# GZHoffie/approximate-string-matching

Measured on AMD Instinct MI355X. Metric: alignments/sec (1e6-pair batch, 100bp, err=0.10) per GPU; NW penalty bit-exact %, higher is better.
Workload: dtype u64; 1 GPU; C2: 1000000 pairs per GPU, len 100-100, err 0.10, k=3, x=o=e=1,1,1, aligners nw+leap+greedy, greedy tails=clean; pairs_per_gpu=1000000

## Files before the change

### approximate-string-matching_amd/csrc/asm_capi.hip

```cpp
#include <hip/hip_runtime.h>
#include <hipcub/hipcub.hpp>
#include <math.h>
#include <stddef.h>
#include <stdio.h>
#include <stdlib.h>
#include <string.h>

#include <algorithm>
#include <atomic>
#include <chrono>
#include <condition_variable>
#include <fcntl.h>
#include <functional>
#include <map>
#include <memory>
#include <mutex>
#include <string>
#include <sys/stat.h>
#include <thread>
#include <type_traits>
#include <unistd.h>
#include <unordered_map>
#include <vector>

#include "../../include/asm_mi355x.h"
#include "asm_host.h"
#include "asm_kernels.h"
#include "asm_greedy3_kernel.h"
#include "asm_wide.h"
#include "asm_wave.h"
#include "asm_group.h"
#include "asm_cover.h"
#include "asm_tails.h"
#include "asm_filter.h"
#include "asm_ingest.h"
#include "asm_map.h"
#include "asm_fastq.h"
#include "asm_sam.h"

struct asm_handle {
    unsigned long long serial = 0;
    int device = 0;
    hipStream_t own_stream = nullptr;
    hipStream_t stream = nullptr;
    unsigned long long* d_pair_queue = nullptr;
    hipStream_t side_stream = nullptr;
    hipStream_t pack_stream = nullptr;
    hipEvent_t ev_packed = nullptr;
    hipEvent_t ev_nw = nullptr;
    hipStream_t acc_stream = nullptr;
    hipEvent_t ev_leap = nullptr, ev_tail = nullptr;
    bool tail_set = false;
    hipEvent_t ev_out[2] = {nullptr, nullptr};
    unsigned calls3 = 0;
    const void* last3_out[3] = {nullptr, nullptr, nullptr};
    bool last3_valid = false;
    bool pipe_prev = false;
    hipEvent_t ev_gate = nullptr;
    bool gate_set = false;
    hipEvent_t ev_fork = nullptr, ev_join = nullptr, ev_switch = nullptr;
    bool overlap = true;
    std::string err;
    int num_cus = 256;
    int refill_greedy = 8;
    bool greedy_fast = true;
    struct G3Table {
        G3Sig sig;
        int k;
        bool ok;
        uint2* d;
    };
    std::vector<G3Table> g3_tables;
    const uint2* d_g3_table = nullptr;
    bool leap_hint = true;
    bool bucketing = true;
    bool wave_kernels = true;
    bool nw_bylen = true;
    bool nw_banded = true;
    bool nw_wfa = true;
    int64_t map_cand_cap = (int64_t)1 << 24;
    int64_t map_chunk = (int64_t)1 << 18;
    int64_t map_run_cap = (int64_t)1 << 24;
    std::vector<hipEvent_t> prof_ev;
    std::vector<unsigned> prof_mask;
    int prof_cap = 0;
    unsigned prof_select = 0xfu;
    void* d_sort = nullptr;
    size_t sort_cap = 0;
    bool leap_sort = true;
    uint32_t* d_todo = nullptr;
    size_t todo_cap = 0;
    std::unordered_map<void*, size_t> pool_live;
    std::multimap<size_t, void*> pool_idle;
    size_t pool_idle_bytes = 0;
    bool pooling = true;
    char* pin_raw[3] = {nullptr, nullptr, nullptr};
    size_t pin_raw_cap = 0;
    int32_t* pin_pen[2][3] = {{nullptr, nullptr, nullptr}, {nullptr, nullptr, nullptr}};
    int64_t pin_pen_cap[2][3] = {{0, 0, 0}, {0, 0, 0}};
};

static size_t pool_round(size_t bytes) {
    if (bytes <= 4096) return 4096;
    int top = 63 - __builtin_clzll((unsigned long long)bytes);
    const size_t step = (size_t)1 << (top - 3);
    return (bytes + step - 1) & ~(step - 1);
}
// ... 221 lines not shown
            hipStreamSynchronize(h->stream) == hipSuccess) {
            t.ok = true;
        } else {
            (void)hipGetLastError();
            if (t.d) (void)hipFree(t.d);
            t.d = nullptr;
        }
    }
    h->g3_tables.push_back(t);
    h->d_g3_table = t.d;
    return t.ok;
}

template <int K>
static hipError_t launch_greedy_fast(asm_handle* h, const asm_bucket& b, const GreedyArgs& ga, OutMap out, CigarSink cig) {
    constexpr int NT = G3_THREADS;
    auto kern = greedy_fast_kernel<K, NT>;
    const size_t lds = g3_lds_bytes(K, NT);
    {
        hipError_t e = hipFuncSetAttribute(reinterpret_cast<const void*>(kern), hipFuncAttributeMaxDynamicSharedMemorySize, (int)lds);
        if (e != hipSuccess) return e;
    }
    int64_t blocks = h->num_cus;
    const int64_t need = (b.n + NT - 1) / NT;
    if (blocks > need) blocks = need;
    const G3Sig sig = {ga.sig_match, ga.sig_mismatch, ga.sig_indel};
    hipLaunchKernelGGL(kern, dim3((unsigned)blocks), dim3(NT), lds, h->stream, (const uint4*)b.planes, (const uint32_t*)b.lens,
                       (long)b.n, b.w4, sig, h->d_g3_table, out, cig, h->refill_greedy);
    return hipGetLastError();
}

template <int K>
static hipError_t launch_greedy(asm_handle* h, const asm_bucket& b, const GreedyArgs& ga, OutMap out, CigarSink cig) {
#ifdef GREEDY_DIAG
    if (cig.ops == nullptr && g_diag_buf) cig.nops = (uint8_t*)g_diag_buf;
#endif
    const bool unit = ga.x == 1 && ga.o == 1 && ga.e == 1 && !ga.semi;
    if constexpr (K <= 3) {
        if (h->greedy_fast && unit && g3_prepare(h, ga, K)) return launch_greedy_fast<K>(h, b, ga, out, cig);
    }
    if (unit)
        return launch_persistent(h, greedy_persist_kernel<K, true>, b.n, (const uint4*)b.planes, (const uint32_t*)b.lens,
                                 (long)b.n, b.w4, ga, out, cig, h->refill_greedy);
    return launch_persistent(h, greedy_persist_kernel<K, false>, b.n, (const uint4*)b.planes, (const uint32_t*)b.lens,
                             (long)b.n, b.w4, ga, out, cig, h->refill_greedy);
}

#define LEAP_UNIT_WIDE_K 5
#define LEAP_UNIT_MAX_K 10
template <int K, int W64>
static hipError_t launch_leap_unit_w(asm_handle* h, const asm_bucket& b, OutMap out, const int32_t* hint) {
    if (hint && h->leap_hint) {
        const unsigned blocks = (unsigned)((b.n + LEAP_HINT_PAIRS - 1) / LEAP_HINT_PAIRS);
        hipLaunchKernelGGL((leap_unit_hint_kernel<K, W64>), dim3(blocks), dim3(ASM_BLOCK), 0, h->stream, b.planes, b.lens,
                           (long)b.n, b.w4, out, hint);
        return hipGetLastError();
    }
    hipLaunchKernelGGL((leap_unit_kernel<K, W64>), dim3(grid_for(b.n)), dim3(ASM_BLOCK), 0, h->stream, b.planes, b.lens,
                       (long)b.n, b.w4, out);
    return hipGetLastError();
}

template <int K, int W64>
static hipError_t launch_leap_general_w(asm_handle* h, const asm_bucket& b, const asm_params* p, OutMap out) {
    const dim3 grid((unsigned)((b.n + LEAP_GEN_THREADS - 1) / LEAP_GEN_THREADS)), block(LEAP_GEN_THREADS);
    const RingGeometry rg(p->x, p->o, p->e);
    const bool bytes = b.maxlen + 4 <= 255 && rg.lds_bytes(2 * K + 1, LEAP_GEN_THREADS, 2) > 20 * 1024;
    if (bytes)
        hipLaunchKernelGGL((leap_general_kernel<K, W64, uint8_t>), grid, block, rg.lds_bytes(2 * K + 1, LEAP_GEN_THREADS, 1), h->stream,
                           b.planes, b.lens, (long)b.n, b.w4, (int)p->x, (int)p->o, (int)p->e, rg.gm, rg.gi, out);
    else
        hipLaunchKernelGGL((leap_general_kernel<K, W64, uint16_t>), grid, block, rg.lds_bytes(2 * K + 1, LEAP_GEN_THREADS, 2), h->stream,
                           b.planes, b.lens, (long)b.n, b.w4, (int)p->x, (int)p->o, (int)p->e, rg.gm, rg.gi, out);
    return hipGetLastError();
}

template <int K, int W64, typename EnT>
static void launch_nw_wfa_pass(asm_handle* h, const asm_bucket& b, const asm_params* p, OutMap out, const uint32_t* in_list,
                               const uint32_t* in_count, uint32_t* todo, uint32_t* todo_count) {
    const WfaRings rg(p->x, p->o, p->e);
    const dim3 grid((unsigned)((b.n + LEAP_GEN_THREADS - 1) / LEAP_GEN_THREADS)), block(LEAP_GEN_THREADS);
    hipLaunchKernelGGL((nw_wfa_kernel<K, W64, EnT, false>), grid, block, rg.lds_bytes(2 * K + 1, LEAP_GEN_THREADS, sizeof(EnT)),
                       h->stream, b.planes, b.lens, (long)b.n, b.w4, (int)p->x, (int)p->o, (int)p->e, rg.gm, rg.gi, out, in_list,
                       in_count, todo, todo_count);
}

template <int W64, int MAXROWS>
static int launch_nw_wfa(asm_handle* h, const asm_bucket& b, const asm_params* p, OutMap out) {
    const size_t words = 2 * ((size_t)b.n + 1);
    if (h->todo_cap < words) {
        if (h->d_todo) (void)hipFree(h->d_todo);
        h->d_todo = nullptr, h->todo_cap = 0;
        HIPCHK(h, big_malloc(h, (void**)&h->d_todo, sizeof(uint32_t) * words));
        h->todo_cap = words;
    }
    uint32_t* const list_a = h->d_todo;
    uint32_t* const list_b = h->d_todo + (size_t)b.n + 1;
    HIPCHK(h, hipMemsetAsync(list_a, 0, sizeof(uint32_t), h->stream));
    HIPCHK(h, hipMemsetAsync(list_b, 0, sizeof(uint32_t), h->stream));
    const WfaRings rg(p->x, p->o, p->e);
    bool bytes = false;
    if constexpr (W64 == 2) {
        bytes = true;
        launch_nw_wfa_pass<NW_WFA_K, 2, uint8_t>(h, b, p, out, nullptr, nullptr, list_a + 1, list_a);
    }
    if (!bytes) launch_nw_wfa_pass<NW_WFA_K, W64, uint16_t>(h, b, p, out, nullptr, nullptr, list_a + 1, list_a);
    const uint32_t* rest = list_a;
    const size_t en = b.maxlen + 2 <= 255 ? 1 : 2;
// ... 127 lines not shown
        SIMD_ED_CASE(1)
        SIMD_ED_CASE(2)
        SIMD_ED_CASE(3)
        SIMD_ED_CASE(4)
        SIMD_ED_CASE(5)
        SIMD_ED_CASE(6)
        SIMD_ED_CASE(7)
        SIMD_ED_CASE(8)
        default: {
            const size_t lds = (size_t)2 * (2 * T + 3) * SIMD_ED_THREADS * sizeof(short);
            hipLaunchKernelGGL((simd_ed_kernel<0, W64>), grid, block, lds, h->stream, b.planes, b.lens, (long)b.n, b.w4, T, shd,
                               ed_mode, ev);
        }
    }
#undef SIMD_ED_CASE
    HIPCHK(h, hipGetLastError());
    return ASM_OK;
}

extern "C" {

const char* asm_version(void) { return "asm_mi355x 0.1 (gfx950)"; }

void asm_default_params(asm_params* p) {
    if (!p) return;
    p->k = 3;
    p->x = p->o = p->e = 1;
    p->p_match = 0.80;
    p->p_mismatch = 0.20 / 3;
    p->p_indel = 0.40 / 3;
    p->alignment_type = ASM_ALIGN_GLOBAL;
    p->leap_mode = ASM_LEAP_GLOBAL;
}

int asm_device_count(void) {
    int c = 0;
    if (hipGetDeviceCount(&c) != hipSuccess) return 0;
    return c;
}

static void handle_teardown(asm_handle* h) {
    (void)hipSetDevice(h->device);
    if (h->own_stream) (void)hipStreamDestroy(h->own_stream);
    if (h->side_stream) (void)hipStreamDestroy(h->side_stream);
    if (h->d_pair_queue) (void)hipFree(h->d_pair_queue);
    if (h->d_sort) (void)hipFree(h->d_sort);
    if (h->pack_stream) (void)hipStreamDestroy(h->pack_stream);
    if (h->ev_packed) (void)hipEventDestroy(h->ev_packed);
    if (h->ev_gate) (void)hipEventDestroy(h->ev_gate);
    if (h->ev_leap) (void)hipEventDestroy(h->ev_leap);
    if (h->ev_tail) (void)hipEventDestroy(h->ev_tail);
    for (hipEvent_t ev : h->ev_out)
        if (ev) (void)hipEventDestroy(ev);
    if (h->acc_stream) (void)hipStreamDestroy(h->acc_stream);
    if (h->ev_nw) (void)hipEventDestroy(h->ev_nw);
    if (h->ev_fork) (void)hipEventDestroy(h->ev_fork);
    if (h->ev_join) (void)hipEventDestroy(h->ev_join);
    if (h->ev_switch) (void)hipEventDestroy(h->ev_switch);
    if (h->d_todo) (void)hipFree(h->d_todo);
    for (auto& t : h->g3_tables)
        if (t.d) (void)hipFree(t.d);
    for (hipEvent_t ev : h->prof_ev) (void)hipEventDestroy(ev);
    (void)hipDeviceSynchronize();
    for (char* q : h->pin_raw)
        if (q) (void)hipHostFree(q);
    for (auto& row : h->pin_pen)
        for (int32_t* q : row)
            if (q) (void)hipHostFree(q);
    pool_release_idle(h);
    for (auto& kv : h->pool_live) (void)hipFree(kv.first);
    delete h;
}

int asm_create(asm_handle** out, int device) {
    if (!out) return fail(nullptr, ASM_EINVAL, "asm_create: out is NULL");
    *out = nullptr;
    int c = 0;
    if (hipGetDeviceCount(&c) != hipSuccess || c <= 0)
        return fail(nullptr, ASM_ENODEVICE, "asm_create: no HIP device is visible (this library has no CPU path)");
    if (device < 0 || device >= c) return fail(nullptr, ASM_EINVAL, "asm_create: device index out of range");
    std::unique_ptr<asm_handle, void (*)(asm_handle*)> owned(new asm_handle, handle_teardown);
    asm_handle* const h = owned.get();
    h->device = device;
    HIPCHK(h, hipSetDevice(device));
    HIPCHK(h, hipStreamCreateWithFlags(&h->own_stream, hipStreamNonBlocking));
    h->stream = h->own_stream;
    HIPCHK(h, hipStreamCreateWithFlags(&h->side_stream, hipStreamNonBlocking));
    HIPCHK(h, hipMalloc((void**)&h->d_pair_queue, sizeof(unsigned long long)));
    HIPCHK(h, hipStreamCreateWithFlags(&h->pack_stream, hipStreamNonBlocking));
    HIPCHK(h, hipEventCreateWithFlags(&h->ev_packed, hipEventDisableTiming));
    HIPCHK(h, hipEventCreateWithFlags(&h->ev_gate, hipEventDisableTiming));
    HIPCHK(h, hipStreamCreateWithFlags(&h->acc_stream, hipStreamNonBlocking));
    HIPCHK(h, hipEventCreateWithFlags(&h->ev_nw, hipEventDisableTiming));
    HIPCHK(h, hipEventCreateWithFlags(&h->ev_leap, hipEventDisableTiming));
    HIPCHK(h, hipEventCreateWithFlags(&h->ev_tail, hipEventDisableTiming));
    for (hipEvent_t& ev : h->ev_out) HIPCHK(h, hipEventCreateWithFlags(&ev, hipEventDisableTiming));
    HIPCHK(h, hipEventCreateWithFlags(&h->ev_fork, hipEventDisableTiming));
    HIPCHK(h, hipEventCreateWithFlags(&h->ev_join, hipEventDisableTiming));
    HIPCHK(h, hipEventCreateWithFlags(&h->ev_switch, hipEventDisableTiming));
    hipDeviceProp_t prop;
    HIPCHK(h, hipGetDeviceProperties(&prop, device));
    h->num_cus = prop.multiProcessorCount > 0 ? prop.multiProcessorCount : 256;
    const char* env;
    if ((env = getenv("ASM_OVERLAP"))) h->overlap = env[0] != '0';
    if ((env = getenv("ASM_LEAP_HINT"))) h->leap_hint = env[0] != '0';
    if ((env = getenv("ASM_LEAP_SORT"))) h->leap_sort = env[0] != '0';
    if ((env = getenv("ASM_BUCKET"))) h->bucketing = env[0] != '0';
    if ((env = getenv("ASM_WAVE"))) h->wave_kernels = env[0] != '0';
    if ((env = getenv("ASM_POOL"))) h->pooling = env[0] != '0';
    if ((env = getenv("ASM_NW_BANDED"))) h->nw_banded = env[0] != '0';
    if ((env = getenv("ASM_NW_BYLEN"))) h->nw_bylen = env[0] != '0';
    if ((env = getenv("ASM_NW_WFA"))) h->nw_wfa = env[0] != '0';
    if ((env = getenv("ASM_GREEDY_FAST"))) h->greedy_fast = env[0] != '0';
    if ((env = getenv("ASM_MAP_CAND_CAP")) && atoll(env) > 0) h->map_cand_cap = atoll(env);
    if ((env = getenv("ASM_MAP_CHUNK")) && atoll(env) > 0) h->map_chunk = atoll(env);
    if ((env = getenv("ASM_MAP_RUN_CAP")) && atoll(env) > 0) h->map_run_cap = atoll(env);
    {
        std::lock_guard<std::mutex> lk(g_live_mu);
        h->serial = g_next_serial++;
        g_live_handles.push_back(h);
    }
    *out = owned.release();
    return ASM_OK;
}

int asm_destroy(asm_handle* h) {
    if (!h) return ASM_OK;
    {
        std::lock_guard<std::mutex> lk(g_live_mu);
        for (size_t i = 0; i < g_live_handles.size(); i++)
            if (g_live_handles[i] == h) {
                g_live_handles.erase(g_live_handles.begin() + (long)i);
                break;
            }
    }
    handle_teardown(h);
    return ASM_OK;
}

const char* asm_last_error(const asm_handle* h) { return h ? h->err.c_str() : g_err.c_str(); }

static int switch_stream(asm_handle* h, hipStream_t next) {
    if (next == h->stream) return ASM_OK;
    HIPCHK(h, hipSetDevice(h->device));
    HIPCHK(h, hipEventRecord(h->ev_switch, h->stream));
    HIPCHK(h, hipStreamWaitEvent(next, h->ev_switch, 0));
    if (h->tail_set) HIPCHK(h, hipStreamWaitEvent(next, h->ev_tail, 0));
    h->stream = next;
    return ASM_OK;
}

int asm_set_stream(asm_handle* h, void* hip_stream) {
    if (!h) return fail(nullptr, ASM_EINVAL, "asm_set_stream: NULL handle");
    return switch_stream(h, (hipStream_t)hip_stream);
}

int asm_reset_stream(asm_handle* h) {
    if (!h) return fail(nullptr, ASM_EINVAL, "asm_reset_stream: NULL handle");
    return switch_stream(h, h->own_stream);
}

int asm_synchronize(asm_handle* h) {
    if (!h) return fail(nullptr, ASM_EINVAL, "asm_synchronize: NULL handle");
    HIPCHK(h, hipSetDevice(h->device));
    HIPCHK(h, hipStreamSynchronize(h->stream));
    if (h->tail_set) HIPCHK(h, hipStreamSynchronize(h->acc_stream));
    return ASM_OK;
}

int asm_pipeline_join_async(asm_handle* h) {
    if (!h) return fail(nullptr, ASM_EINVAL, "asm_pipeline_join_async: NULL handle");
    HIPCHK(h, hipSetDevice(h->device));
    if (h->tail_set) HIPCHK(h, hipStreamWaitEvent(h->stream, h->ev_tail, 0));
    h->pipe_prev = false;
    h->last3_valid = false;
    return ASM_OK;
}

static int check_gen(const asm_gen_config* cfg) {
    std::string err;
    const int rc = asm_host::check_gen(cfg, err);
    return rc ? fail(nullptr, rc, err) : ASM_OK;
}

int asm_generate_pairs(const asm_gen_config* cfg, int64_t first, int64_t n, uint32_t* read_off, uint32_t* ref_off,
                       char* reads, size_t reads_cap, char* refs, size_t refs_cap) {
    std::string err;
    const int rc = asm_host::generate_pairs(cfg, first, n, read_off, ref_off, reads, reads_cap, refs, refs_cap, err);
    return rc ? fail(nullptr, rc, err) : ASM_OK;
}


static hipError_t launch_pack(asm_handle* h, const asm_batch* b, const uint4* tails, uint4* planes, uint32_t* lens,
                              const PackBuckets& pb, const uint32_t* pos) {
    const dim3 grid((unsigned)((b->n + PACK_BLOCK - 1) / PACK_BLOCK)), block(PACK_BLOCK);
    int wmax = 1;
    for (int q = 0; q < pb.nb; q++) wmax = pb.w4[q] > wmax ? pb.w4[q] : wmax;
    const auto side_dwords = [](size_t bytes) { return (size_t)2 * (size_t)(((bytes + 15) / 16 + 1) / 2 + 1); };
    size_t dw = 2 * side_dwords((size_t)PACK_BLOCK * (size_t)b->maxlen + 15);
    if (dw > PACK_LDS_MAX / 4) dw = PACK_LDS_MAX / 4;
    if (dw < side_dwords((size_t)b->maxlen + 30)) dw = side_dwords((size_t)b->maxlen + 30);
#define PACK_LAUNCH(W)                                                                                                   \
    hipLaunchKernelGGL((pack_kernel<W>), grid, block, dw * 4, h->stream, b->d_reads, b->d_read_off, b->d_refs,           \
                       b->d_ref_off, tails, planes, lens, (long)b->n, pb, pos, (uint32_t)dw)
    switch (wmax) {
        case 1: PACK_LAUNCH(1); break;
        case 2: PACK_LAUNCH(2); break;
        case 3: PACK_LAUNCH(3); break;
        default: PACK_LAUNCH(4); break;
    }
#undef PACK_LAUNCH
    return hipGetLastError();
}

int asm_batch_pack_async(asm_handle* h, asm_batch* b) {
    if (!h || !b) return fail(h, ASM_EINVAL, "asm_batch_pack_async: NULL argument");
    if (b->n == 0) return ASM_OK;
    HIPCHK(h, hipSetDevice(h->device));
    HIPCHK(h, launch_pack(h, b, b->d_tails, b->d_planes, b->d_lens, b->pb, b->d_pos));
    return ASM_OK;
}

static int batch_resolve_tails(asm_handle* h, asm_batch* b, const uint8_t* init256, uint8_t* summary256, bool emit) {
    if (summary256) memset(summary256, TAIL_NONE, 256);
    if (b->n == 0) return ASM_OK;
    const long nchunks = (b->n + TAIL_CHUNK - 1) / TAIL_CHUNK;
// ... 341 lines not shown
        HIPCHK(h, hipMemcpy(refs, b->d_refs, b->refs_bytes, hipMemcpyDeviceToHost));
    }
    return ASM_OK;
}

int64_t asm_batch_planes_size(const asm_batch* b) { return b ? (int64_t)b->planes_total : 0; }

int asm_batch_download_planes(asm_handle* h, const asm_batch* b, uint32_t* planes, size_t planes_cap, uint32_t* lens,
                              uint32_t* order) {
    if (!h || !b) return fail(h, ASM_EINVAL, "asm_batch_download_planes: NULL argument");
    HIPCHK(h, hipSetDevice(h->device));
    HIPCHK(h, hipStreamSynchronize(h->stream));
    const size_t n = (size_t)b->n;
    if (planes) {
        if (planes_cap < 4 * b->planes_total) return fail(h, ASM_EINVAL, "asm_batch_download_planes: planes buffer too small");
        HIPCHK(h, hipMemcpy(planes, b->d_planes, sizeof(uint4) * b->planes_total, hipMemcpyDeviceToHost));
    }
    if (lens && n) HIPCHK(h, hipMemcpy(lens, b->d_lens, sizeof(uint32_t) * n, hipMemcpyDeviceToHost));
    if (order && n) {
        if (b->d_order) HIPCHK(h, hipMemcpy(order, b->d_order, sizeof(uint32_t) * n, hipMemcpyDeviceToHost));
        else
            for (size_t i = 0; i < n; i++) order[i] = (uint32_t)i;
    }
    return ASM_OK;
}

static int check_params(asm_handle* h, int aligner, const asm_params* p, int maxlen = ASM_MAX_LENGTH) {
    if (!p) return fail(h, ASM_EINVAL, "params is NULL");
    if (p->x < 0 || p->o < 0 || p->e < 0) return fail(h, ASM_EINVAL, "penalties must be non-negative");
    if (aligner == ASM_GREEDY) {
        if (p->k < 0 || p->k > ASM_GREEDY_MAX_K) return fail(h, ASM_EINVAL, "Greedy: k must be in [0, 50] (MAX_K, hurdle_matrix.h:8)");
        if (!(p->p_match > 0 && p->p_mismatch > 0 && p->p_indel > 0)) return fail(h, ASM_EINVAL, "Greedy: probabilities must be positive");
        if (p->alignment_type != ASM_ALIGN_GLOBAL && p->alignment_type != ASM_ALIGN_SEMI_GLOBAL)
            return fail(h, ASM_EUNSUPPORTED, "Greedy: alignment type must be GLOBAL or SEMI_GLOBAL (LOCAL is unsupported in the reference too, hurdle_matrix.h:467)");
    } else if (aligner == ASM_LEAP) {
        if (p->k < 0 || p->k > ASM_WIDE_MAX_K) return fail(h, ASM_EINVAL, "LEAP: k out of range");
        if (p->x < 1 || p->o < 1 || p->e < 1 || p->o < p->e)
            return fail(h, ASM_EINVAL, "LEAP: need x >= 1, o >= e >= 1 (LV_BAG.cpp:165-166)");
        if (p->x > ASM_WIDE_MAX_PENALTY || p->o > ASM_WIDE_MAX_PENALTY)
            return fail(h, ASM_EUNSUPPORTED, "LEAP: penalties above the compiled history depth");
        if (p->leap_mode < ASM_LEAP_GLOBAL || p->leap_mode > ASM_LEAP_SEMI_FREE_END)
            return fail(h, ASM_EINVAL, "LEAP: leap_mode must be one of ASM_LEAP_GLOBAL/LOCAL/SEMI_FREE_BEGIN/SEMI_FREE_END");
        if (p->leap_mode != ASM_LEAP_GLOBAL && maxlen > 512)
            return fail(h, ASM_EUNSUPPORTED, "LEAP: the non-GLOBAL modes are built for strings up to 512 characters");
    } else if (aligner == ASM_NW) {
        const long worst = 2L * ((long)p->o + (long)(maxlen > 0 ? maxlen - 1 : 0) * (long)p->e) + (long)p->o;
        if (p->x > 10000 || p->o > 10000 || p->e > 10000 || worst >= (long)NW_BIG)
            return fail(h, ASM_EUNSUPPORTED, "NW: penalties too large for this batch's longest sequence "
                                             "(need 2*(o + (maxlen-1)*e) + o < 30000 and x, o, e <= 10000)");
    } else {
        return fail(h, ASM_EINVAL, "unknown aligner id");
    }
    return ASM_OK;
}

static int align_bucket(asm_handle* h, const asm_bucket& b, int aligner, const asm_params* p, OutMap out,
                        CigarSink cig = CigarSink{nullptr, nullptr, 0}, const int32_t* hint = nullptr) {
    if (b.n == 0) return ASM_OK;
    const bool unit = (p->x == 1 && p->o == 1 && p->e == 1);
    const uint4* planes = b.planes;
    const uint32_t* lens = b.lens;
    if (aligner == ASM_GREEDY) {
        GreedyArgs ga;
        ga.x = p->x, ga.o = p->o, ga.e = p->e;
        ga.semi = p->alignment_type == ASM_ALIGN_SEMI_GLOBAL ? 1 : 0;
        ga.sig_match = log(p->p_match / 0.25);
        ga.sig_mismatch = log(p->p_mismatch / 0.25);
        ga.sig_indel = log(p->p_indel / 2 / 0.25);
        switch (p->k) {
            case 1: HIPCHK(h, launch_greedy<1>(h, b, ga, out, cig)); break;
            case 2: HIPCHK(h, launch_greedy<2>(h, b, ga, out, cig)); break;
            case 3: HIPCHK(h, launch_greedy<3>(h, b, ga, out, cig)); break;
            case 4: HIPCHK(h, launch_greedy<4>(h, b, ga, out, cig)); break;
            case 5: HIPCHK(h, launch_greedy<5>(h, b, ga, out, cig)); break;
#define GREEDY_WIDE_CASE(KK) \
            case KK: HIPCHK(h, launch_greedy<KK>(h, b, ga, out, cig)); break;
            GREEDY_WIDE_CASE(6) GREEDY_WIDE_CASE(7) GREEDY_WIDE_CASE(8) GREEDY_WIDE_CASE(9) GREEDY_WIDE_CASE(10) GREEDY_WIDE_CASE(11)
            GREEDY_WIDE_CASE(12) GREEDY_WIDE_CASE(13) GREEDY_WIDE_CASE(14) GREEDY_WIDE_CASE(15) GREEDY_WIDE_CASE(16)
#undef GREEDY_WIDE_CASE
            default:
                if (h->wave_kernels && p->k >= 32 && p->k <= 39 && (long)p->o + 110L * p->e < 16000L) {
                    HIPCHK(h, launch_greedy_group(h->stream, planes, lens, b.n, b.w4, (int)p->k, ga, out, cig, h->num_cus));
                } else if (p->k <= ASM_WAVE_MAX_K && h->wave_kernels && unit && !ga.semi) {
                    HIPCHK(h, hipMemsetAsync(h->d_pair_queue, 0, sizeof(unsigned long long), h->stream));
                    launch_wave_per_pair(h->stream, greedy_wave_kernel<true>, b.n, h->num_cus, planes, lens, (long)b.n, b.w4,
                                         (int)p->k, ga, out, cig, h->d_pair_queue, (const uint32_t*)nullptr, (const uint32_t*)nullptr);
                } else if (p->k <= ASM_WAVE_MAX_K && h->wave_kernels && (long)p->o + 62L * p->e < 16000L) {
                    HIPCHK(h, hipMemsetAsync(h->d_pair_queue, 0, sizeof(unsigned long long), h->stream));
                    launch_wave_per_pair(h->stream, greedy_wave_kernel<false>, b.n, h->num_cus, planes, lens, (long)b.n, b.w4,
                                         (int)p->k, ga, out, cig, h->d_pair_queue, (const uint32_t*)nullptr, (const uint32_t*)nullptr);
                } else if (h->wave_kernels && (long)p->o + 100L * p->e < 16000L)
                    launch_greedy_wave2(h->stream, planes, lens, b.n, b.w4, (int)p->k, ga, out, cig, h->num_cus);
                else
                    launch_greedy_wide(h->stream, planes, lens, b.n, b.w4, p->k, ga, out, cig);
                break;
        }
    } else if (aligner == ASM_LEAP) {
        if (p->leap_mode != ASM_LEAP_GLOBAL) {
            launch_leap_wide(h->stream, planes, lens, b.n, b.w4, p->k, p->x, p->o, p->e, out, (int)p->leap_mode);
        } else if (unit && p->k >= 1 && ((p->k <= LEAP_UNIT_WIDE_K && b.maxlen <= 384) || (p->k <= LEAP_UNIT_MAX_K && b.maxlen <= 128))) {
            switch (p->k) {
                case 1: HIPCHK(h, launch_leap_unit<1>(h, b, out, hint)); break;
                case 2: HIPCHK(h, launch_leap_unit<2>(h, b, out, hint)); break;
                case 3: HIPCHK(h, launch_leap_unit<3>(h, b, out, hint)); break;
                case 4: HIPCHK(h, launch_leap_unit<4>(h, b, out, hint)); break;
                case 5: HIPCHK(h, launch_leap_unit<5>(h, b, out, hint)); break;
                case 6: HIPCHK(h, launch_leap_unit<6>(h, b, out, hint)); break;
                case 7: HIPCHK(h, launch_leap_unit<7>(h, b, out, hint)); break;
                case 8: HIPCHK(h, launch_leap_unit<8>(h, b, out, hint)); break;
                case 9: HIPCHK(h, launch_leap_unit<9>(h, b, out, hint)); break;
                default: HIPCHK(h, launch_leap_unit<10>(h, b, out, hint)); break;
            }
        } else if (!unit && p->k >= 1 && ((p->k <= 5 && b.maxlen <= 256) || (p->k <= 8 && b.maxlen <= 128)) && h->wave_kernels &&
                   RingGeometry(p->x, p->o, p->e).lds_bytes(2 * p->k + 1, LEAP_GEN_THREADS) <= 64 * 1024) {
            switch (p->k) {
                case 1: HIPCHK(h, launch_leap_general<1>(h, b, p, out)); break;
                case 2: HIPCHK(h, launch_leap_general<2>(h, b, p, out)); break;
                case 3: HIPCHK(h, launch_leap_general<3>(h, b, p, out)); break;
                case 4: HIPCHK(h, launch_leap_general<4>(h, b, p, out)); break;
                case 5: HIPCHK(h, launch_leap_general<5>(h, b, p, out)); break;
                case 6: HIPCHK(h, launch_leap_general<6>(h, b, p, out)); break;
                case 7: HIPCHK(h, launch_leap_general<7>(h, b, p, out)); break;
                default: HIPCHK(h, launch_leap_general<8>(h, b, p, out)); break;
            }
        } else if (h->wave_kernels && b.maxlen <= 512 &&
                   leap_quad_lds((b.maxlen + 31) / 32, (int)p->k, unit ? 2 : RingGeometry(p->x, p->o, p->e).gm,
                                 unit ? 0 : RingGeometry(p->x, p->o, p->e).gi, b.maxlen + 2 <= 255 ? 1 : 2) <= 64 * 1024) {
            const RingGeometry rg(p->x, p->o, p->e);
            const int w32 = (b.maxlen + 31) / 32;
            const int32_t* const qhint = h->leap_hint ? hint : nullptr;
            const uint32_t* qperm = nullptr;
            if (qhint && h->leap_sort && (b.maxlen > 128 || !unit)) {
                const size_t n = (size_t)b.n;
                size_t tmp_bytes = 0;
                HIPCHK(h, hipcub::DeviceRadixSort::SortPairs(nullptr, tmp_bytes, (uint8_t*)nullptr, (uint8_t*)nullptr, (uint32_t*)nullptr,
                                                             (uint32_t*)nullptr, (int)n, 0, 6, h->stream));
                const size_t need = 2 * n + 8 * n + tmp_bytes + 256;
                if (h->sort_cap < need) {
                    if (h->d_sort) (void)hipFree(h->d_sort);
                    h->d_sort = nullptr, h->sort_cap = 0;
                    HIPCHK(h, big_malloc(h, (void**)&h->d_sort, need));
                    h->sort_cap = need;
                }
                uint32_t* const d_idx = (uint32_t*)h->d_sort;
                uint32_t* const d_perm = d_idx + n;
                uint8_t* const d_keys = (uint8_t*)(d_perm + n);
                uint8_t* const d_keys2 = d_keys + n;
                void* const d_tmp = (void*)(((uintptr_t)(d_keys2 + n) + 255) & ~(uintptr_t)255);
                const int div = unit ? 1 : (int)(p->e < p->x ? p->e : p->x);
                hipLaunchKernelGGL(leap_sort_keys_kernel, dim3((unsigned)((n + 255) / 256)), dim3(256), 0, h->stream, qhint, out, (long)n,
                                   div, d_keys, d_idx);
                HIPCHK(h, hipcub::DeviceRadixSort::SortPairs(d_tmp, tmp_bytes, d_keys, d_keys2, d_idx, d_perm, (int)n, 0, 6, h->stream));
                qperm = d_perm;
// ... 432 lines not shown
        return fail(h, ASM_EINVAL, "asm_run_benchmark_async: repack = 3 needs output arrays that alternate between two sets (these "
                                   "were the previous call's); asm_pipeline_join_async first to reuse them");
    if (repack != 3) h->last3_valid = false, h->calls3 = 0;
    if (repack != 3 && h->tail_set) {
        HIPCHK(h, hipSetDevice(h->device));
        HIPCHK(h, hipStreamWaitEvent(main_stream, h->ev_tail, 0));
        h->tail_set = false;
    }
    bool pipelined = false;
    if ((repack == 2 || repack == 3) && b->n > 0) {
        HIPCHK(h, hipSetDevice(h->device));
        if (!b->d_planes_alt) HIPCHK(h, batch_alloc(b, &b->d_planes_alt, sizeof(uint4) * b->planes_total));
        if (!b->d_lens_alt) HIPCHK(h, batch_alloc(b, &b->d_lens_alt, sizeof(uint32_t) * (size_t)b->n));
        if (!b->ev_consumed[1]) {
            for (hipEvent_t& ev : b->ev_consumed)
                if (!ev) HIPCHK(h, hipEventCreateWithFlags(&ev, hipEventDisableTiming));
            HIPCHK(h, hipEventRecord(b->ev_consumed[0], main_stream));
            HIPCHK(h, hipEventRecord(b->ev_consumed[1], main_stream));
        }
        HIPCHK(h, hipStreamWaitEvent(h->pack_stream, b->ev_consumed[b->cur ^ 1], 0));
        if (repack == 3 && h->calls3 >= 2) HIPCHK(h, hipStreamWaitEvent(h->pack_stream, h->ev_out[h->calls3 & 1u], 0));
        if (!h->pipe_prev) {
            HIPCHK(h, hipEventRecord(h->ev_fork, main_stream));
            HIPCHK(h, hipStreamWaitEvent(h->pack_stream, h->ev_fork, 0));
        }
        if (h->gate_set && repack == 2) HIPCHK(h, hipStreamWaitEvent(h->pack_stream, h->ev_gate, 0));
        PROF(0, 0, h->pack_stream)
        batch_flip_planes(b);
        h->stream = h->pack_stream;
        rc = asm_batch_pack_async(h, b);
        h->stream = main_stream;
        if (rc) batch_flip_planes(b);
        PROF(0, 1, h->pack_stream)
        if (!rc) {
            HIPCHK(h, hipEventRecord(h->ev_packed, h->pack_stream));
            HIPCHK(h, hipStreamWaitEvent(main_stream, h->ev_packed, 0));
        }
        pipelined = true;
    } else if (repack) {
        PROF(0, 0, main_stream)
        rc = asm_batch_pack_async(h, b);
        PROF(0, 1, main_stream)
    }
    const bool greedy_first = greedy_first_shape && !rc;
    if (greedy_first) {
        PROF(3, 0, main_stream)
        rc = asm_align_batch_async(h, b, ASM_GREEDY, p, d_greedy);
        PROF(3, 1, main_stream)
    }
    if (repack == 3 && pipelined && !rc) {
        h->last3_out[0] = d_nw, h->last3_out[1] = d_leap, h->last3_out[2] = d_greedy;
        h->last3_valid = true;
        hipEvent_t out_free = h->ev_out[h->calls3 & 1u];
        if (h->calls3 >= 2) {
            HIPCHK(h, hipStreamWaitEvent(main_stream, out_free, 0));
            if (d_greedy) HIPCHK(h, hipStreamWaitEvent(h->side_stream, out_free, 0));
        }
        if (d_greedy) {
            hipStream_t side = h->side_stream;
            HIPCHK(h, hipStreamWaitEvent(side, h->ev_packed, 0));
            PROF(3, 0, side)
            h->stream = side;
            rc = asm_align_batch_async(h, b, ASM_GREEDY, p, d_greedy);
            h->stream = main_stream;
            PROF(3, 1, side)
            if (!rc) HIPCHK(h, hipEventRecord(h->ev_join, side));
        }
        hipStream_t chain = (d_nw && d_leap) ? h->acc_stream : main_stream;
        if (chain != main_stream) HIPCHK(h, hipStreamWaitEvent(chain, h->ev_packed, 0));
        if (!rc && d_nw) {
            PROF(1, 0, chain)
            h->stream = chain;
            rc = asm_align_batch_async(h, b, ASM_NW, p, d_nw);
            h->stream = main_stream;
            PROF(1, 1, chain)
        }
        hipStream_t ls = (d_nw && d_leap) ? h->acc_stream : main_stream;
        if (!rc && d_leap) {
            if (ls != chain) {
                HIPCHK(h, hipEventRecord(h->ev_nw, chain));
                HIPCHK(h, hipStreamWaitEvent(ls, h->ev_nw, 0));
            }
            PROF(2, 0, ls)
            h->stream = ls;
            rc = asm_align_batch_hinted_async(h, b, ASM_LEAP, p, d_nw, d_leap);
            h->stream = main_stream;
            PROF(2, 1, ls)
        }
        if (pe) h->prof_mask.push_back(pmask);
        if (rc) return rc;
        HIPCHK(h, hipEventRecord(h->ev_leap, ls));
        HIPCHK(h, hipStreamWaitEvent(h->acc_stream, h->ev_leap, 0));
        if (d_greedy) HIPCHK(h, hipStreamWaitEvent(h->acc_stream, h->ev_join, 0));
        if (d_counters) {
            h->stream = h->acc_stream;
            rc = asm_accuracy_async(h, d_nw, d_leap, d_greedy, d_answers, b->n, d_counters);
            h->stream = main_stream;
            if (rc) return rc;
        }
        HIPCHK(h, hipEventRecord(b->ev_consumed[b->cur], h->acc_stream));
        HIPCHK(h, hipEventRecord(out_free, h->acc_stream));
        h->calls3++;
        HIPCHK(h, hipEventRecord(h->ev_tail, h->acc_stream));
        h->tail_set = true;
        h->pipe_prev = true;
        return ASM_OK;
    }
    const bool fork = h->overlap && d_greedy && (d_nw || d_leap) && !rc && !greedy_first;
    if (fork) {
        HIPCHK(h, hipEventRecord(h->ev_fork, main_stream));
        HIPCHK(h, hipStreamWaitEvent(h->side_stream, h->ev_fork, 0));
        PROF(3, 0, h->side_stream)
        h->stream = h->side_stream;
        rc = asm_align_batch_async(h, b, ASM_GREEDY, p, d_greedy);
        h->stream = main_stream;
        PROF(3, 1, h->side_stream)
        if (!rc) HIPCHK(h, hipEventRecord(h->ev_join, h->side_stream));
    }
    if (!rc && d_nw) {
        PROF(1, 0, main_stream)
        rc = asm_align_batch_async(h, b, ASM_NW, p, d_nw);
        PROF(1, 1, main_stream)
        if (!rc && repack == 2) {
            HIPCHK(h, hipEventRecord(h->ev_gate, main_stream));
            h->gate_set = true;
        }
    }
    if (!rc && d_leap) {
        PROF(2, 0, main_stream)
        rc = asm_align_batch_hinted_async(h, b, ASM_LEAP, p, greedy_first ? d_greedy : d_nw, d_leap);
        PROF(2, 1, main_stream)
    }
    if (fork) {
        if (!rc) HIPCHK(h, hipStreamWaitEvent(main_stream, h->ev_join, 0));
    } else if (!rc && d_greedy && !greedy_first) {
        PROF(3, 0, main_stream)
        rc = asm_align_batch_async(h, b, ASM_GREEDY, p, d_greedy);
        PROF(3, 1, main_stream)
    }
#undef PROF
    if (pe) h->prof_mask.push_back(pmask);
    if (pipelined && !rc) HIPCHK(h, hipEventRecord(b->ev_consumed[b->cur], main_stream));
    if (!rc && d_counters) rc = asm_accuracy_async(h, d_nw, d_leap, d_greedy, d_answers, b->n, d_counters);
    h->pipe_prev = pipelined;
    return rc;
}

#include "asm_stream.h"

namespace {
using asm_host::NlScan;
using asm_host::scan_newlines;

static int batch_from_device_text(asm_handle* h, const char* d_raw, size_t nbytes, asm_batch* b) {
    const int64_t n = b->n;
    const size_t cnt = (size_t)n + 1;
// ... 306 lines not shown
```

### approximate-string-matching_amd/csrc/asm_kernels.h

```cpp
#pragma once
#include <hip/hip_runtime.h>
#include <stdint.h>

#include "asm_bits.h"
#include "asm_gen.h"

#define ASM_BLOCK 256

#ifndef PACK_BLOCK
#define PACK_BLOCK 256
#endif
#define PACK_LDS_MAX (33 * 1024)
#define PACK_UNROLL 8

struct PackBuckets {
    int nb;
    int w4[4];
    long start[5];
    long plane_off[4];
};

ASM_DEV uint32_t swar_zero_bytes(uint32_t t) {
    return ~(((t & 0x7f7f7f7fu) + 0x7f7f7f7fu) | t | 0x7f7f7f7fu);
}
// ... 531 lines not shown
#pragma unroll
    for (int j = 0; j < NL; j++) above[j] = vw_above<W64>(mask[j]);

    int result = -1;
    {
        int e0 = vw_next_one<W64>(mask[K], 0);
        e0 = e0 > len ? len : e0;
        en[K] = e0;
        if (e0 == len) result = 0;
    }
    for (int e = 1; e <= ASM_LEAP_AF_THRESHOLD && result < 0; e++) {
        int en2[NL];
        bool pass = false;
#pragma unroll
        for (int j = 0; j < NL; j++) {
            const int d = j - K;
            const int top = d >= 0 ? 1 : 0, bot = d <= 0 ? 1 : 0;
            const int e_up = j > 0 ? en[j - 1] : -2;
            const int e_dn = j < NL - 1 ? en[j + 1] : -2;
            int st = en[j] + 1;
            st = e_up + top > st ? e_up + top : st;
            st = e_dn + bot > st ? e_dn + bot : st;
            int enew = -2;
            if (st >= 0) {
                const int from = st > len ? len : st;
                int t = VW_SCAN_FB(W64) ? vw_next_one_fb<W64>(mask[j], above[j], from) : vw_next_one<W64>(mask[j], from);
                t = t > len ? len : t;
                enew = t > st ? t : st;
                if (enew == len) {
                    const int diff = d < 0 ? -d : d;
                    const int conv = e + diff;
                    if (conv <= ASM_LEAP_AF_THRESHOLD) pass = true;
                }
            }
            en2[j] = enew;
        }
#pragma unroll
        for (int j = 0; j < NL; j++) en[j] = en2[j];
        if (pass) result = e;
    }
    return result;
}

template <int K, int W64>
__global__ __launch_bounds__(ASM_BLOCK) void leap_unit_kernel(const uint4* __restrict__ planes,
                                                              const uint32_t* __restrict__ lens, long n, int w4,
                                                              OutMap out) {
    const long i = (long)blockIdx.x * blockDim.x + threadIdx.x;
    if (i >= n) return;
    out.put(i, leap_unit_pair<K, W64>(planes, lens, n, w4, i));
}

#define LEAP_HINT_PAIRS 256
template <int K, int W64>
__global__ __launch_bounds__(ASM_BLOCK) void leap_unit_hint_kernel(const uint4* __restrict__ planes,
                                                                   const uint32_t* __restrict__ lens, long n, int w4,
                                                                   OutMap out, const int32_t* __restrict__ hint) {
    __shared__ uint16_t s_sorted[LEAP_HINT_PAIRS];
    __shared__ int s_bin[64];
    const int t = threadIdx.x;
    const long base = (long)blockIdx.x * LEAP_HINT_PAIRS;
    const int cnt = (n - base) < LEAP_HINT_PAIRS ? (int)(n - base) : LEAP_HINT_PAIRS;
    if (t < 64) s_bin[t] = 0;
    __syncthreads();
    int key[LEAP_HINT_PAIRS / ASM_BLOCK];
#pragma unroll
    for (int q = 0; q < LEAP_HINT_PAIRS / ASM_BLOCK; q++) {
        const int local = t + q * ASM_BLOCK;
        key[q] = -1;
        if (local < cnt) {
            int h = hint[out.index(base + local)];
            h = h < 0 ? 63 : (h > 63 ? 63 : h);
            key[q] = h;
            atomicAdd(&s_bin[h], 1);
        }
    }
    __syncthreads();
    if (t == 0) {
        int run = 0;
        for (int b = 0; b < 64; b++) {
            const int c = s_bin[b];
            s_bin[b] = run;
            run += c;
        }
    }
    __syncthreads();
#pragma unroll
    for (int q = 0; q < LEAP_HINT_PAIRS / ASM_BLOCK; q++) {
        if (key[q] >= 0) {
            const int slot = atomicAdd(&s_bin[key[q]], 1);
            s_sorted[slot] = (uint16_t)(t + q * ASM_BLOCK);
        }
    }
    __syncthreads();
    for (int q = 0; q < LEAP_HINT_PAIRS / ASM_BLOCK; q++) {
        const int p = t + q * ASM_BLOCK;
        if (p < cnt) {
            const long i = base + s_sorted[p];
            out.put(i, leap_unit_pair<K, W64>(planes, lens, n, w4, i));
        }
    }
}

#define LEAP_GEN_THREADS 128
struct RingGeometry {
    int gm, gi;
    __host__ __device__ static int pow2_above(int v) {
        int g = 2;
        while (g <= v) g <<= 1;
        return g;
    }
    __host__ RingGeometry(int x, int o, int e) : gm(pow2_above(x > o ? x : o)), gi(pow2_above(e)) {}
    __host__ size_t lds_bytes(int nl, int threads, size_t elem = sizeof(short)) const { return ((size_t)(gm + 2 * gi) * nl * threads * elem + 3) & ~(size_t)3; }
};

template <int K, int W64, typename EnT>
__global__ __launch_bounds__(LEAP_GEN_THREADS) void leap_general_kernel(const uint4* __restrict__ planes,
                                                                        const uint32_t* __restrict__ lens, long n, int w4,
                                                                        int x, int o, int ext, int gm, int gi, OutMap out) {
    constexpr int NL = 2 * K + 1, T = LEAP_GEN_THREADS, SLOT = NL * T;
    extern __shared__ uint32_t s_ring32[];
    const int t = threadIdx.x;
    EnT* const r_en = reinterpret_cast<EnT*>(s_ring32) + t;
    EnT* const r_ip = r_en + gm * SLOT;
    EnT* const r_dp = r_ip + gi * SLOT;
    const long i = (long)blockIdx.x * T + t;
    if (i >= n) return;
    const uint32_t ln = lens[i];
    const int m = (int)(ln & 0xffffu), nn = (int)(ln >> 16);
    const int len = m > nn ? m : nn;
    VW<W64> A0, A1, B0, B1;
    load_planes<W64>(planes, n, w4, i, A0, A1, B0, B1);
    const VW<W64> VA = vw_low_ones<W64>(m), VB = vw_low_ones<W64>(nn);
    VW<W64> mask[NL];
#pragma unroll
    for (int j = 0; j < NL; j++) mask[j] = leap_lane_mask<W64>(A0, A1, B0, B1, VA, VB, j - K);
    VWAbove<W64> above[NL];
#pragma unroll
    for (int j = 0; j < NL; j++) above[j] = vw_above<W64>(mask[j]);

    int result = -1;
#pragma unroll
    for (int j = 0; j < NL; j++) {
        for (int q = 0; q < gm; q++) r_en[q * SLOT + j * T] = (EnT)0;
        for (int q = 0; q < gi; q++) r_ip[q * SLOT + j * T] = (EnT)0, r_dp[q * SLOT + j * T] = (EnT)0;
    }
    {
        int e0 = vw_next_one<W64>(mask[K], 0);
        e0 = e0 > len ? len : e0;
        r_en[K * T] = (EnT)(e0 + 2);
        if (e0 == len) result = 0;
    }
    for (int e = 1; e <= ASM_LEAP_AF_THRESHOLD && result < 0; e++) {
        const EnT* const en_o = r_en + ((e - o) & (gm - 1)) * SLOT;
// ... 534 lines not shown
    const long stride = (long)gridDim.x * blockDim.x;
    unsigned int c_nw = 0, c_leap = 0, c_greedy = 0;
    const long n4 = (nw != nullptr || answers != nullptr) ? n >> 2 : 0;
    const long n_cmp = (nw != nullptr || answers != nullptr) ? n : 0;
    const int4* nw4 = reinterpret_cast<const int4*>(nw);
    const int4* leap4 = reinterpret_cast<const int4*>(leap);
    const int4* greedy4 = reinterpret_cast<const int4*>(greedy);
    const int4* ans4 = reinterpret_cast<const int4*>(answers);
    constexpr int ACC_AHEAD = 4;
    for (long q0 = i; q0 < n4; q0 += ACC_AHEAD * stride) {
        int4 p[ACC_AHEAD], a[ACC_AHEAD], l[ACC_AHEAD], g[ACC_AHEAD];
#pragma unroll
        for (int u = 0; u < ACC_AHEAD; u++) {
            const long q = q0 + u * stride;
            const long qq = q < n4 ? q : q0;
            p[u] = a[u] = l[u] = g[u] = make_int4(INT32_MIN, INT32_MIN, INT32_MIN, INT32_MIN);
            if (nw != nullptr) p[u] = nw4[qq];
            if (answers != nullptr) a[u] = ans4[qq];
            if (leap != nullptr) l[u] = leap4[qq];
            if (greedy != nullptr) g[u] = greedy4[qq];
        }
#pragma unroll
        for (int u = 0; u < ACC_AHEAD; u++) {
            if (q0 + u * stride >= n4) break;
            int4 want = p[u];
            if (answers != nullptr) {
                want.x = a[u].x != INT32_MIN ? a[u].x : p[u].x, want.y = a[u].y != INT32_MIN ? a[u].y : p[u].y;
                want.z = a[u].z != INT32_MIN ? a[u].z : p[u].z, want.w = a[u].w != INT32_MIN ? a[u].w : p[u].w;
            }
            if (nw != nullptr) c_nw += (p[u].x == want.x) + (p[u].y == want.y) + (p[u].z == want.z) + (p[u].w == want.w);
            if (leap != nullptr) c_leap += (l[u].x == want.x) + (l[u].y == want.y) + (l[u].z == want.z) + (l[u].w == want.w);
            if (greedy != nullptr) c_greedy += (g[u].x == want.x) + (g[u].y == want.y) + (g[u].z == want.z) + (g[u].w == want.w);
        }
    }
    for (long r = (n4 << 2) + i; r < n_cmp; r += stride) {
        const int32_t p = nw != nullptr ? nw[r] : INT32_MIN;
        int32_t want = p;
        if (answers != nullptr && answers[r] != INT32_MIN) want = answers[r];
        if (nw != nullptr) c_nw += (p == want) ? 1u : 0u;
        if (leap != nullptr) c_leap += (leap[r] == want) ? 1u : 0u;
        if (greedy != nullptr) c_greedy += (greedy[r] == want) ? 1u : 0u;
    }
    const unsigned int t_nw = block_sum_256(c_nw, s_part);
    const unsigned int t_leap = block_sum_256(c_leap, s_part);
    const unsigned int t_greedy = block_sum_256(c_greedy, s_part);
    if (threadIdx.x == 0) {
        if (blockIdx.x == 0) atomicAdd(&counters[0], (unsigned long long)n);
        if (t_nw) atomicAdd(&counters[1], (unsigned long long)t_nw);
        if (t_leap) atomicAdd(&counters[2], (unsigned long long)t_leap);
        if (t_greedy) atomicAdd(&counters[3], (unsigned long long)t_greedy);
    }
}

__global__ __launch_bounds__(ASM_BLOCK) void gen_lengths_kernel(asm_gen_config cfg, long first, long n,
                                                                uint32_t* __restrict__ mlen,
                                                                uint32_t* __restrict__ nlen) {
    const long i = (long)blockIdx.x * blockDim.x + threadIdx.x;
    if (i >= n) return;
    int m, nn;
    asm_gen_lengths(&cfg, (uint64_t)(first + i), &m, &nn);
    mlen[i] = (uint32_t)m;
    nlen[i] = (uint32_t)nn;
}

__global__ __launch_bounds__(64) void gen_fill_kernel(asm_gen_config cfg, long first, long n,
                                                      const uint32_t* __restrict__ read_off,
                                                      const uint32_t* __restrict__ ref_off,
                                                      char* __restrict__ reads, char* __restrict__ refs) {
    const long i = (long)blockIdx.x * blockDim.x + threadIdx.x;
    if (i >= n) return;
    char rd[ASM_MAX_LENGTH + 8];
    char tx[ASM_GEN_MAX_TEXT];
    int m, nn;
    asm_gen_pair(&cfg, (uint64_t)(first + i), rd, tx, &m, &nn);
    char* r = reads + read_off[i];
    char* t = refs + ref_off[i];
    for (int j = 0; j < m; j++) r[j] = rd[j];
    for (int j = 0; j < nn; j++) t[j] = tx[j];
}
```

Before: 5.259 billion read pairs/s through NW+Leap+Greedy (whole job; consecutive steps overlap, inputs rotate over resident batches; value_in_order = the same steps strictly in order).

## Fuse accuracy counting into LEAP hint kernel with per-block partials and fold

The accuracy comparison (NW/LEAP/greedy vs answers) is folded into the LEAP hint kernel, which writes per-block partial counts. A single-block fold kernel then sums them into the global counters. This removes a separate full pass over the three output arrays on the acc stream. In exchange, LEAP now has to wait for greedy to finish (ev_join) before it starts, and the tail moves onto the main stream, which may reduce overlap between steps.

Result: slower. 5.128 billion read pairs/s through NW+Leap+Greedy (whole job; consecutive steps overlap, inputs rotate over resident batches; value_in_order = the same steps strictly in order) (-2.5%).

```diff
diff --git a/approximate-string-matching_amd/csrc/asm_capi.hip b/approximate-string-matching_amd/csrc/asm_capi.hip
--- a/approximate-string-matching_amd/csrc/asm_capi.hip
+++ b/approximate-string-matching_amd/csrc/asm_capi.hip
@@ -52,7 +52,15 @@
     hipEvent_t ev_leap = nullptr, ev_tail = nullptr;
     bool tail_set = false;
     hipEvent_t ev_out[2] = {nullptr, nullptr};
+    hipEvent_t ev_fold[2] = {nullptr, nullptr};
+    bool fold_rec[2] = {false, false};
     unsigned calls3 = 0;
+    bool fuse_counters = true;
+    uint32_t* d_partials[2] = {nullptr, nullptr};
+    size_t partials_cap[2] = {0, 0};
+    std::vector<void*> partials_retired;
+    const LeapCount* leap_count = nullptr;
+    bool leap_count_used = false;
     const void* last3_out[3] = {nullptr, nullptr, nullptr};
     bool last3_valid = false;
     bool pipe_prev = false;
@@ -380,8 +388,13 @@
 static hipError_t launch_leap_unit_w(asm_handle* h, const asm_bucket& b, OutMap out, const int32_t* hint) {
     if (hint && h->leap_hint) {
         const unsigned blocks = (unsigned)((b.n + LEAP_HINT_PAIRS - 1) / LEAP_HINT_PAIRS);
-        hipLaunchKernelGGL((leap_unit_hint_kernel<K, W64>), dim3(blocks), dim3(ASM_BLOCK), 0, h->stream, b.planes, b.lens,
-                           (long)b.n, b.w4, out, hint);
+        if (h->leap_count) {
+            hipLaunchKernelGGL((leap_unit_hint_count_kernel<K, W64>), dim3(blocks), dim3(ASM_BLOCK), 0, h->stream, b.planes,
+                               b.lens, (long)b.n, b.w4, out, hint, *h->leap_count);
+            h->leap_count_used = true;
+        } else
+            hipLaunchKernelGGL((leap_unit_hint_kernel<K, W64>), dim3(blocks), dim3(ASM_BLOCK), 0, h->stream, b.planes, b.lens,
+                               (long)b.n, b.w4, out, hint);
         return hipGetLastError();
     }
     hipLaunchKernelGGL((leap_unit_kernel<K, W64>), dim3(grid_for(b.n)), dim3(ASM_BLOCK), 0, h->stream, b.planes, b.lens,
@@ -615,6 +628,8 @@
     if (h->ev_tail) (void)hipEventDestroy(h->ev_tail);
     for (hipEvent_t ev : h->ev_out)
         if (ev) (void)hipEventDestroy(ev);
+    for (hipEvent_t ev : h->ev_fold)
+        if (ev) (void)hipEventDestroy(ev);
     if (h->acc_stream) (void)hipStreamDestroy(h->acc_stream);
     if (h->ev_nw) (void)hipEventDestroy(h->ev_nw);
     if (h->ev_fork) (void)hipEventDestroy(h->ev_fork);
@@ -625,6 +640,8 @@
         if (t.d) (void)hipFree(t.d);
     for (hipEvent_t ev : h->prof_ev) (void)hipEventDestroy(ev);
     (void)hipDeviceSynchronize();
+    for (uint32_t* q : h->d_partials) pool_free(h, q);
+    for (void* q : h->partials_retired) pool_free(h, q);
     for (char* q : h->pin_raw)
         if (q) (void)hipHostFree(q);
     for (auto& row : h->pin_pen)
@@ -658,6 +675,7 @@
     HIPCHK(h, hipEventCreateWithFlags(&h->ev_leap, hipEventDisableTiming));
     HIPCHK(h, hipEventCreateWithFlags(&h->ev_tail, hipEventDisableTiming));
     for (hipEvent_t& ev : h->ev_out) HIPCHK(h, hipEventCreateWithFlags(&ev, hipEventDisableTiming));
+    for (hipEvent_t& ev : h->ev_fold) HIPCHK(h, hipEventCreateWithFlags(&ev, hipEventDisableTiming));
     HIPCHK(h, hipEventCreateWithFlags(&h->ev_fork, hipEventDisableTiming));
     HIPCHK(h, hipEventCreateWithFlags(&h->ev_join, hipEventDisableTiming));
     HIPCHK(h, hipEventCreateWithFlags(&h->ev_switch, hipEventDisableTiming));
@@ -675,6 +693,7 @@
     if ((env = getenv("ASM_NW_BYLEN"))) h->nw_bylen = env[0] != '0';
     if ((env = getenv("ASM_NW_WFA"))) h->nw_wfa = env[0] != '0';
     if ((env = getenv("ASM_GREEDY_FAST"))) h->greedy_fast = env[0] != '0';
+    if ((env = getenv("ASM_FUSE_COUNTERS"))) h->fuse_counters = env[0] != '0';
     if ((env = getenv("ASM_MAP_CAND_CAP")) && atoll(env) > 0) h->map_cand_cap = atoll(env);
     if ((env = getenv("ASM_MAP_CHUNK")) && atoll(env) > 0) h->map_chunk = atoll(env);
     if ((env = getenv("ASM_MAP_RUN_CAP")) && atoll(env) > 0) h->map_run_cap = atoll(env);
@@ -735,6 +754,8 @@
     if (!h) return fail(nullptr, ASM_EINVAL, "asm_pipeline_join_async: NULL handle");
     HIPCHK(h, hipSetDevice(h->device));
     if (h->tail_set) HIPCHK(h, hipStreamWaitEvent(h->stream, h->ev_tail, 0));
+    for (void* q : h->partials_retired) pool_free(h, q);
+    h->partials_retired.clear();
     h->pipe_prev = false;
     h->last3_valid = false;
     return ASM_OK;
@@ -1182,6 +1203,12 @@
         return fail(h, ASM_EINVAL, "unknown aligner id");
     }
     return ASM_OK;
+}
+
+static bool leap_unit_shape(const asm_bucket& b, const asm_params* p) {
+    const bool unit = (p->x == 1 && p->o == 1 && p->e == 1);
+    return p->leap_mode == ASM_LEAP_GLOBAL && unit && p->k >= 1 &&
+           ((p->k <= LEAP_UNIT_WIDE_K && b.maxlen <= 384) || (p->k <= LEAP_UNIT_MAX_K && b.maxlen <= 128));
 }
 
 static int align_bucket(asm_handle* h, const asm_bucket& b, int aligner, const asm_params* p, OutMap out,
@@ -1228,7 +1255,7 @@
     } else if (aligner == ASM_LEAP) {
         if (p->leap_mode != ASM_LEAP_GLOBAL) {
             launch_leap_wide(h->stream, planes, lens, b.n, b.w4, p->k, p->x, p->o, p->e, out, (int)p->leap_mode);
-        } else if (unit && p->k >= 1 && ((p->k <= LEAP_UNIT_WIDE_K && b.maxlen <= 384) || (p->k <= LEAP_UNIT_MAX_K && b.maxlen <= 128))) {
+        } else if (leap_unit_shape(b, p)) {
             switch (p->k) {
                 case 1: HIPCHK(h, launch_leap_unit<1>(h, b, out, hint)); break;
                 case 2: HIPCHK(h, launch_leap_unit<2>(h, b, out, hint)); break;
@@ -1767,6 +1794,16 @@
         h->last3_out[0] = d_nw, h->last3_out[1] = d_leap, h->last3_out[2] = d_greedy;
         h->last3_valid = true;
         hipEvent_t out_free = h->ev_out[h->calls3 & 1u];
+        const unsigned set = h->calls3 & 1u;
+        const bool fuse = h->fuse_counters && d_nw && d_leap && d_greedy && d_counters && b->nb == 1 && !b->bk[0].order &&
+                          h->leap_hint && leap_unit_shape(b->bk[0], p);
+        const size_t fold_blocks = (size_t)((b->n + LEAP_HINT_PAIRS - 1) / LEAP_HINT_PAIRS);
+        if (fuse && h->partials_cap[set] < fold_blocks) {
+            uint32_t* fresh = nullptr;
+            HIPCHK(h, pool_alloc(h, (void**)&fresh, sizeof(uint32_t) * 4 * fold_blocks));
+            if (h->d_partials[set]) h->partials_retired.push_back(h->d_partials[set]);
+            h->d_partials[set] = fresh, h->partials_cap[set] = fold_blocks;
+        }
         if (h->calls3 >= 2) {
             HIPCHK(h, hipStreamWaitEvent(main_stream, out_free, 0));
             if (d_greedy) HIPCHK(h, hipStreamWaitEvent(h->side_stream, out_free, 0));
@@ -1796,27 +1833,45 @@
                 HIPCHK(h, hipEventRecord(h->ev_nw, chain));
                 HIPCHK(h, hipStreamWaitEvent(ls, h->ev_nw, 0));
             }
+            const LeapCount lc = {d_greedy, d_answers, h->d_partials[set]};
+            if (fuse) {
+                HIPCHK(h, hipStreamWaitEvent(ls, h->ev_join, 0));
+                if (h->fold_rec[set]) HIPCHK(h, hipStreamWaitEvent(ls, h->ev_fold[set], 0));
+                h->leap_count = &lc, h->leap_count_used = false;
+            }
             PROF(2, 0, ls)
             h->stream = ls;
             rc = asm_align_batch_hinted_async(h, b, ASM_LEAP, p, d_nw, d_leap);
             h->stream = main_stream;
+            h->leap_count = nullptr;
             PROF(2, 1, ls)
+            if (!rc && fuse && !h->leap_count_used)
+                rc = fail(h, ASM_EINVAL, "asm_run_benchmark_async: LEAP did not take the counting kernel (internal error)");
         }
         if (pe) h->prof_mask.push_back(pmask);
         if (rc) return rc;
         HIPCHK(h, hipEventRecord(h->ev_leap, ls));
-        HIPCHK(h, hipStreamWaitEvent(h->acc_stream, h->ev_leap, 0));
-        if (d_greedy) HIPCHK(h, hipStreamWaitEvent(h->acc_stream, h->ev_join, 0));
-        if (d_counters) {
-            h->stream = h->acc_stream;
-            rc = asm_accuracy_async(h, d_nw, d_leap, d_greedy, d_answers, b->n, d_counters);
-            h->stream = main_stream;
-            if (rc) return rc;
-        }
-        HIPCHK(h, hipEventRecord(b->ev_consumed[b->cur], h->acc_stream));
-        HIPCHK(h, hipEventRecord(out_free, h->acc_stream));
+        hipStream_t tail = fuse ? main_stream : h->acc_stream;
+        HIPCHK(h, hipStreamWaitEvent(tail, h->ev_leap, 0));
+        if (fuse) {
+            hipLaunchKernelGGL(counters_fold_kernel, dim3(1), dim3(ASM_BLOCK), 0, tail, (const uint32_t*)h->d_partials[set],
+                               (long)fold_blocks, (long)b->n, d_counters);
+            HIPCHK(h, hipGetLastError());
+            HIPCHK(h, hipEventRecord(h->ev_fold[set], tail));
+            h->fold_rec[set] = true;
+        } else {
+            if (d_greedy) HIPCHK(h, hipStreamWaitEvent(tail, h->ev_join, 0));
+            if (d_counters) {
+                h->stream = tail;
+                rc = asm_accuracy_async(h, d_nw, d_leap, d_greedy, d_answers, b->n, d_counters);
+                h->stream = main_stream;
+                if (rc) return rc;
+            }
+        }
+        HIPCHK(h, hipEventRecord(b->ev_consumed[b->cur], tail));
+        HIPCHK(h, hipEventRecord(out_free, tail));
         h->calls3++;
-        HIPCHK(h, hipEventRecord(h->ev_tail, h->acc_stream));
+        HIPCHK(h, hipEventRecord(h->ev_tail, tail));
         h->tail_set = true;
         h->pipe_prev = true;
         return ASM_OK;
diff --git a/approximate-string-matching_amd/csrc/asm_kernels.h b/approximate-string-matching_amd/csrc/asm_kernels.h
--- a/approximate-string-matching_amd/csrc/asm_kernels.h
+++ b/approximate-string-matching_amd/csrc/asm_kernels.h
@@ -607,10 +607,15 @@
 }
 
 #define LEAP_HINT_PAIRS 256
-template <int K, int W64>
-__global__ __launch_bounds__(ASM_BLOCK) void leap_unit_hint_kernel(const uint4* __restrict__ planes,
-                                                                   const uint32_t* __restrict__ lens, long n, int w4,
-                                                                   OutMap out, const int32_t* __restrict__ hint) {
+struct LeapCount {
+    const int32_t* greedy;
+    const int32_t* answers;
+    uint32_t* partials;
+};
+
+template <int K, int W64, bool COUNT>
+ASM_DEV void leap_unit_hint_body(const uint4* __restrict__ planes, const uint32_t* __restrict__ lens, long n, int w4,
+                                 OutMap out, const int32_t* __restrict__ hint, LeapCount cnt_args) {
     __shared__ uint16_t s_sorted[LEAP_HINT_PAIRS];
     __shared__ int s_bin[64];
     const int t = threadIdx.x;
@@ -648,13 +653,60 @@
         }
     }
     __syncthreads();
+    unsigned int c_nw = 0, c_leap = 0, c_greedy = 0;
     for (int q = 0; q < LEAP_HINT_PAIRS / ASM_BLOCK; q++) {
         const int p = t + q * ASM_BLOCK;
+        bool ok_nw = false, ok_leap = false, ok_greedy = false;
         if (p < cnt) {
             const long i = base + s_sorted[p];
-            out.put(i, leap_unit_pair<K, W64>(planes, lens, n, w4, i));
-        }
-    }
+            const int leap = leap_unit_pair<K, W64>(planes, lens, n, w4, i);
+            out.put(i, leap);
+            if constexpr (COUNT) {
+                const int32_t nw = hint[i];
+                int32_t want = nw;
+                if (cnt_args.answers != nullptr) {
+                    const int32_t a = cnt_args.answers[i];
+                    want = a != INT32_MIN ? a : nw;
+                }
+                ok_nw = nw == want, ok_leap = leap == want, ok_greedy = cnt_args.greedy[i] == want;
+            }
+        }
+        if constexpr (COUNT) {
+            c_nw += (unsigned int)__popcll(__ballot(ok_nw));
+            c_leap += (unsigned int)__popcll(__ballot(ok_leap));
+            c_greedy += (unsigned int)__popcll(__ballot(ok_greedy));
+        }
+    }
+    if constexpr (COUNT) {
+        __shared__ unsigned int s_cnt[3][ASM_BLOCK / 64];
+        if ((t & 63) == 0) s_cnt[0][t >> 6] = c_nw, s_cnt[1][t >> 6] = c_leap, s_cnt[2][t >> 6] = c_greedy;
+        __syncthreads();
+        if (t == 0) {
+            unsigned int tot[3];
+#pragma unroll
+            for (int c = 0; c < 3; c++) {
+                tot[c] = 0;
+                for (int w = 0; w < ASM_BLOCK / 64; w++) tot[c] += s_cnt[c][w];
+            }
+            uint32_t* const dst = cnt_args.partials + 4 * (size_t)blockIdx.x;
+            dst[0] = tot[0], dst[1] = tot[1], dst[2] = tot[2];
+        }
+    }
+}
+
+template <int K, int W64>
+__global__ __launch_bounds__(ASM_BLOCK) void leap_unit_hint_kernel(const uint4* __restrict__ planes,
+                                                                   const uint32_t* __restrict__ lens, long n, int w4,
+                                                                   OutMap out, const int32_t* __restrict__ hint) {
+    leap_unit_hint_body<K, W64, false>(planes, lens, n, w4, out, hint, LeapCount{nullptr, nullptr, nullptr});
+}
+
+template <int K, int W64>
+__global__ __launch_bounds__(ASM_BLOCK) void leap_unit_hint_count_kernel(const uint4* __restrict__ planes,
+                                                                         const uint32_t* __restrict__ lens, long n, int w4,
+                                                                         OutMap out, const int32_t* __restrict__ hint,
+                                                                         LeapCount cnt_args) {
+    leap_unit_hint_body<K, W64, true>(planes, lens, n, w4, out, hint, cnt_args);
 }
 
 #define LEAP_GEN_THREADS 128
@@ -1295,6 +1347,31 @@
     }
 }
 
+__global__ __launch_bounds__(ASM_BLOCK) void counters_fold_kernel(const uint32_t* __restrict__ partials, long blocks, long n,
+                                                                  unsigned long long* __restrict__ counters) {
+    __shared__ unsigned long long s_sum[3][ASM_BLOCK / 64];
+    unsigned long long c[3] = {0ull, 0ull, 0ull};
+    for (long b = threadIdx.x; b < blocks; b += ASM_BLOCK) {
+#pragma unroll
+        for (int q = 0; q < 3; q++) c[q] += partials[4 * b + q];
+    }
+#pragma unroll
+    for (int q = 0; q < 3; q++) {
+        for (int off = 32; off > 0; off >>= 1) c[q] += __shfl_down(c[q], off, 64);
+        if ((threadIdx.x & 63) == 0) s_sum[q][threadIdx.x >> 6] = c[q];
+    }
+    __syncthreads();
+    if (threadIdx.x == 0) {
+        atomicAdd(&counters[0], (unsigned long long)n);
+#pragma unroll
+        for (int q = 0; q < 3; q++) {
+            unsigned long long tot = 0ull;
+            for (int w = 0; w < ASM_BLOCK / 64; w++) tot += s_sum[q][w];
+            if (tot) atomicAdd(&counters[1 + q], tot);
+        }
+    }
+}
+
 __global__ __launch_bounds__(ASM_BLOCK) void gen_lengths_kernel(asm_gen_config cfg, long first, long n,
                                                                 uint32_t* __restrict__ mlen,
                                                                 uint32_t* __restrict__ nlen) {
```
